# lambdazy/lzy

Measured on AMD Instinct MI355X. Metric: workflow_makespan_s_8stage_dag, lower is better.
Workload: dtype bf16; 1 GPU; global_batch=8192, seq_len=4096, parallelism=dag-fanout1, ops_per_dag=7, transfers=0, chain_dispatches=2400, stream_plans=0

## Files before the change

### lzy_amd/config.py

```python
from __future__ import annotations

import os
import threading
from dataclasses import dataclass, field, fields
from typing import Any, Dict, Optional


def _coerce(value: str, typ: type) -> Any:
    if typ is bool:
        return value.strip().lower() in ("1", "true", "yes", "on")
    if typ is int:
        return int(value)
    if typ is float:
        return float(value)
    return value


@dataclass
class Config:

    storage: str = ""
    channel_transport: str = "rccl"
    channel_chunk_mb: int = 256
    channel_wire_cast: str = ""
    channel_bundles: bool = True
    bundle_wire_cast: str = ""
    stream_merge: bool = True
    stream_chunk_mb: int = 32
    stream_wire_cast: str = ""
    hip_max_blocks: int = 0
    op_streams: int = 4
    dispatch_workers: int = 0
    exec_threads: int = 2
    chain_dispatch: bool = True
    gang_timeout_s: float = 120.0
    heartbeat_period_s: float = 2.0
    task_retries: int = 1
    settle_wait_s: float = 120.0
    ack_wait_s: float = 300.0
    cache_enabled: bool = True
    journal_ttl_hours: float = 168.0
    keep_hot_max: int = 10000
    spill_enabled: bool = True
    spill_threshold_frac: float = 0.85
    log_archive: bool = True
    log_stream_period_s: float = 0.25
    metrics_port: int = 0
    status_port: int = 0
    user: str = ""

    _frozen_env: Dict[str, str] = field(default_factory=dict, repr=False)

    @staticmethod
    def _load_yaml() -> Dict[str, Any]:
        path = os.environ.get("LZY_CONFIG") or (
            "lzy.yaml" if os.path.exists("lzy.yaml") else ""
        )
        if not path or not os.path.exists(path):
            return {}
        import yaml

        with open(path) as f:
            data = yaml.safe_load(f) or {}
        if not isinstance(data, dict):
            raise ValueError(f"config file {path} must hold a mapping")
        return data

    @classmethod
    def resolve(cls, **overrides: Any) -> "Config":
        data: Dict[str, Any] = {}
        yaml_data = cls._load_yaml()
        for f in fields(cls):
            if f.name.startswith("_"):
                continue
            if f.name in yaml_data:
                data[f.name] = yaml_data[f.name]
            env_key = f"LZY_{f.name.upper()}"
            if env_key in os.environ:
                data[f.name] = _coerce(os.environ[env_key], f.type if isinstance(f.type, type) else type(f.default))
            if f.name in overrides and overrides[f.name] is not None:
                data[f.name] = overrides[f.name]
        if "storage" not in data and os.environ.get("LZY_AMD_STORAGE"):
            data["storage"] = os.environ["LZY_AMD_STORAGE"]
# ... 46 lines not shown
```

### lzy_amd/ops/__init__.py

```python
from __future__ import annotations

import ctypes
import os
from typing import Optional

from lzy_amd.exceptions import NativeExtensionMissing

_LIB_PATH = os.path.join(os.path.dirname(__file__), "libhipops.so")

_lib: Optional[ctypes.CDLL] = None
_load_error: Optional[str] = None
_MX8 = False
_MX8_AXPBY = False
_SEGCOPY = False
SEGCOPY_TILE = 16384
_SEGCODEC = False
SEGCODEC_TILE_ELEMS = 8192
SEGCODEC_RAW = 0
SEGCODEC_ENCODE = 1
SEGCODEC_DECODE = 4


def _try_load() -> Optional[ctypes.CDLL]:
    global _lib, _load_error
    if _lib is not None:
        return _lib
    if not os.path.exists(_LIB_PATH):
        _load_error = f"{_LIB_PATH} not built"
        return None
    try:
        import torch

        torch_hip = os.path.join(
            os.path.dirname(torch.__file__), "lib", "libamdhip64.so"
        )
        if os.path.exists(torch_hip):
            ctypes.CDLL(torch_hip, mode=ctypes.RTLD_GLOBAL)
        lib = ctypes.CDLL(_LIB_PATH)
    except OSError as e:
        _load_error = str(e)
        return None
    lib.lz_cast_copy.restype = ctypes.c_int
    lib.lz_cast_copy.argtypes = [
        ctypes.c_void_p, ctypes.c_int, ctypes.c_void_p, ctypes.c_int,
        ctypes.c_int64, ctypes.c_void_p,
    ]
    lib.lz_checksum.restype = ctypes.c_int
    lib.lz_checksum.argtypes = [
        ctypes.c_void_p, ctypes.c_int64, ctypes.c_void_p, ctypes.c_void_p,
    ]
    lib.lz_checksum_mfma.restype = ctypes.c_int
    lib.lz_checksum_mfma.argtypes = [
        ctypes.c_void_p, ctypes.c_int64, ctypes.c_void_p, ctypes.c_void_p,
    ]
    lib.lz_fill_pattern.restype = ctypes.c_int
    lib.lz_fill_pattern.argtypes = [
        ctypes.c_void_p, ctypes.c_int64, ctypes.c_uint64, ctypes.c_void_p,
    ]
    lib.lz_fill_pattern_masked.restype = ctypes.c_int
    lib.lz_fill_pattern_masked.argtypes = [
        ctypes.c_void_p, ctypes.c_int64, ctypes.c_uint64, ctypes.c_uint64,
        ctypes.c_void_p,
    ]
    lib.lz_stats.restype = ctypes.c_int
    lib.lz_stats.argtypes = [
        ctypes.c_void_p, ctypes.c_int, ctypes.c_int64, ctypes.c_int,
        ctypes.c_void_p, ctypes.c_void_p,
    ]
    lib.lz_stats_variant.restype = ctypes.c_int
    lib.lz_stats_variant.argtypes = [
        ctypes.c_void_p, ctypes.c_int, ctypes.c_int64, ctypes.c_int,
        ctypes.c_void_p, ctypes.c_void_p, ctypes.c_int,
    ]
# ... 19 lines not shown
        ctypes.c_void_p,
    ]
    global _MX8
    try:
        lib.lz_mx8_pack.restype = ctypes.c_int
        lib.lz_mx8_pack.argtypes = [
            ctypes.c_void_p, ctypes.c_int, ctypes.c_void_p, ctypes.c_int64,
            ctypes.c_void_p,
        ]
        lib.lz_mx8_unpack.restype = ctypes.c_int
        lib.lz_mx8_unpack.argtypes = [
            ctypes.c_void_p, ctypes.c_void_p, ctypes.c_int, ctypes.c_int64,
            ctypes.c_void_p,
        ]
        _MX8 = True
    except AttributeError:
        _MX8 = False
    global _MX8_AXPBY
    try:
        lib.lz_mx8_axpby.restype = ctypes.c_int
        lib.lz_mx8_axpby.argtypes = [
            ctypes.c_void_p, ctypes.c_int, ctypes.c_void_p, ctypes.c_void_p,
            ctypes.c_int, ctypes.c_int64, ctypes.c_float, ctypes.c_float,
            ctypes.c_void_p,
        ]
        _MX8_AXPBY = True
    except AttributeError:
        _MX8_AXPBY = False
    global _SEGCOPY
    try:
        lib.lz_segcopy.restype = ctypes.c_int
        lib.lz_segcopy.argtypes = [
            ctypes.c_void_p, ctypes.c_int64, ctypes.c_int64, ctypes.c_int,
            ctypes.c_void_p,
        ]
        lib.lz_segcopy_tile.restype = ctypes.c_int
        lib.lz_segcopy_tile.argtypes = []
        _SEGCOPY = lib.lz_segcopy_tile() == SEGCOPY_TILE
    except AttributeError:
        _SEGCOPY = False
    global _SEGCODEC
    try:
        lib.lz_segcodec.restype = ctypes.c_int
        lib.lz_segcodec.argtypes = [
            ctypes.c_void_p, ctypes.c_int64, ctypes.c_int64, ctypes.c_int,
            ctypes.c_void_p,
        ]
        lib.lz_segcodec_tile_elems.restype = ctypes.c_int
        lib.lz_segcodec_tile_elems.argtypes = []
        _SEGCODEC = _SEGCOPY and \
            lib.lz_segcodec_tile_elems() == SEGCODEC_TILE_ELEMS
    except AttributeError:
        _SEGCODEC = False
    lib.lz_error_name.restype = ctypes.c_char_p
    lib.lz_error_name.argtypes = [ctypes.c_int]
    lib.lz_set_max_blocks.restype = None
    lib.lz_set_max_blocks.argtypes = [ctypes.c_int]
    cap = os.environ.get("LZY_HIP_MAX_BLOCKS")
    if cap:
        lib.lz_set_max_blocks(int(cap))
    _lib = lib
    return lib


NATIVE = _try_load() is not None


def _require_native() -> ctypes.CDLL:
    lib = _try_load()
    if lib is None:
        raise NativeExtensionMissing(
            f"lzy_amd HIP ops not available ({_load_error}); build with "
            f"`python setup.py build_ext --inplace` / __graft_entry__.build() "
            f"(hipcc --offload-arch=gfx950)"
        )
    return lib


def _check(err: int) -> None:
    if err != 0:
        lib = _require_native()
        name = lib.lz_error_name(err).decode()
        raise RuntimeError(f"hipops kernel failed: {name} ({err})")


def _dtype_code(dtype) -> int:
    import torch

    codes = {
        torch.float32: 0,
        torch.float16: 1,
        torch.bfloat16: 2,
        torch.float8_e4m3fn: 3,
        torch.float8_e5m2: 4,
        torch.uint8: 5,
        torch.int32: 6,
        torch.int64: 7,
        torch.float64: 8,
    }
    if dtype not in codes:
        raise ValueError(f"unsupported dtype for hipops: {dtype}")
    return codes[dtype]


def _current_stream_ptr() -> int:
    import torch

    return torch.cuda.current_stream().cuda_stream


def _check_dst(op: str, dst, numel: int, shape=None) -> None:
    if not dst.is_cuda:
        raise ValueError(f"{op}: dst must be a device tensor")
    if not dst.is_contiguous():
        raise ValueError(f"{op}: dst must be contiguous")
    if dst.numel() != numel:
        raise ValueError(
            f"{op}: dst has {dst.numel()} elements, expected {numel}"
        )
    if shape is not None and tuple(dst.shape) != tuple(shape):
        raise ValueError(
            f"{op}: dst has shape {tuple(dst.shape)}, expected {tuple(shape)}"
        )


def cast_copy(src, dst) -> None:
    lib = _require_native()
    if src.numel() != dst.numel():
        raise ValueError("cast_copy: numel mismatch")
    if not (src.is_cuda and dst.is_cuda):
        raise ValueError("cast_copy: device tensors required")
    _check_dst("cast_copy", dst, src.numel())
    s = src.detach().contiguous()
    _check(
        lib.lz_cast_copy(
            ctypes.c_void_p(s.data_ptr()),
            _dtype_code(s.dtype),
            ctypes.c_void_p(dst.data_ptr()),
            _dtype_code(dst.dtype),
            s.numel(),
            ctypes.c_void_p(_current_stream_ptr()),
        )
    )


def _require_mx8() -> ctypes.CDLL:
    lib = _require_native()
    if not _MX8:
        raise NativeExtensionMissing(
            f"{_LIB_PATH} is stale: it lacks lz_mx8_pack/lz_mx8_unpack; "
            f"rebuild with `python setup.py build_ext --inplace --force`"
        )
    return lib


def mx8_nbytes(numel: int) -> int:
    return 33 * ((int(numel) + 31) // 32)


def _mx8_check_dtype(dtype, what: str) -> None:
    import torch

    if dtype not in (torch.float32, torch.bfloat16, torch.float16):
        raise ValueError(f"{what}: dtype must be f32/bf16/f16, got {dtype}")


def mx8_pack(t, out=None):
    import torch

    if not t.is_cuda:
        raise ValueError("mx8_pack requires a device tensor")
    _mx8_check_dtype(t.dtype, "mx8_pack")
    lib = _require_mx8()
    s = t.detach().contiguous()
    n = s.numel()
    nbytes = mx8_nbytes(n)
    if out is None:
        out = torch.empty(nbytes, dtype=torch.uint8, device=s.device)
    elif not (out.is_cuda and out.dtype == torch.uint8 and out.is_contiguous()
              and out.numel() == nbytes):
        raise ValueError(
            f"mx8_pack: out must be a contiguous device uint8[{nbytes}]"
        )
    _check(
        lib.lz_mx8_pack(
            ctypes.c_void_p(s.data_ptr()),
            _dtype_code(s.dtype),
            ctypes.c_void_p(out.data_ptr()),
            n,
            ctypes.c_void_p(_current_stream_ptr()),
        )
    )
    return out


def mx8_unpack(buf, numel_or_shape, dtype, out=None):
    import torch

    if isinstance(numel_or_shape, int):
        shape = (numel_or_shape,)
    else:
        shape = tuple(int(d) for d in numel_or_shape)
    n = 1
    for d in shape:
        n *= d
    if not buf.is_cuda:
        raise ValueError("mx8_unpack requires a device buffer")
    _mx8_check_dtype(dtype, "mx8_unpack")
    if buf.dtype != torch.uint8 or not buf.is_contiguous() \
            or buf.numel() != mx8_nbytes(n):
        raise ValueError(
            f"mx8_unpack: buffer must be contiguous uint8[{mx8_nbytes(n)}] "
            f"for {n} elements, got {buf.dtype}[{buf.numel()}]"
        )
    lib = _require_mx8()
    if out is None:
        out = torch.empty(shape, dtype=dtype, device=buf.device)
    elif not (out.is_cuda and out.dtype == dtype and out.is_contiguous()
              and out.numel() == n):
        raise ValueError(
            f"mx8_unpack: out must be a contiguous device {dtype}[{n}]"
        )
    _check(
        lib.lz_mx8_unpack(
            ctypes.c_void_p(buf.data_ptr()),
            ctypes.c_void_p(out.data_ptr()),
            _dtype_code(dtype),
            n,
            ctypes.c_void_p(_current_stream_ptr()),
        )
    )
    return out


def mx8_axpby(a, wire, alpha: float = 1.0, beta: float = 1.0, dst=None):
    import torch

    if not (a.is_cuda and wire.is_cuda):
        raise ValueError("mx8_axpby requires device tensors")
    _mx8_check_dtype(a.dtype, "mx8_axpby")
    n = a.numel()
    if wire.dtype != torch.uint8 or not wire.is_contiguous() \
            or wire.numel() != mx8_nbytes(n):
        raise ValueError(
            f"mx8_axpby: wire must be contiguous uint8[{mx8_nbytes(n)}] "
            f"for {n} elements, got {wire.dtype}[{wire.numel()}]"
        )
    if dst is not None:
        _check_dst("mx8_axpby", dst, n)
        _mx8_check_dtype(dst.dtype, "mx8_axpby dst")
    lib = _require_native()
    if not _MX8_AXPBY:
        raise NativeExtensionMissing(
            f"{_LIB_PATH} is stale: it lacks lz_mx8_axpby; "
            f"rebuild with `python setup.py build_ext --inplace --force`"
        )
    x = a.detach().contiguous()
    if dst is None:
        dst = torch.empty_like(x)
    _check(
        lib.lz_mx8_axpby(
            ctypes.c_void_p(x.data_ptr()),
            _dtype_code(x.dtype),
            ctypes.c_void_p(wire.data_ptr()),
            ctypes.c_void_p(dst.data_ptr()),
            _dtype_code(dst.dtype),
            n,
            ctypes.c_float(alpha),
            ctypes.c_float(beta),
            ctypes.c_void_p(_current_stream_ptr()),
        )
    )
    return dst



def _require_segcopy() -> ctypes.CDLL:
    lib = _require_native()
    if not _SEGCOPY:
        raise NativeExtensionMissing(
            f"{_LIB_PATH} is stale: it lacks lz_segcopy (tile {SEGCOPY_TILE}); "
            f"rebuild with `python setup.py build_ext --inplace --force`"
        )
    return lib


def _check_align(align: int) -> int:
    align = int(align)
    if align < 1 or align & (align - 1):
        raise ValueError(f"align must be a positive power of two, got {align}")
    return align


def segcopy_layout(sizes, align: int = 128):
    align = _check_align(align)
    offsets = []
    end = 0
    for n in sizes:
        n = int(n)
        if n < 0:
            raise ValueError(f"negative segment size {n}")
        off = (end + align - 1) // align * align
        offsets.append(off)
        end = off + n
    return offsets, (end + align - 1) // align * align


def segcopy_nbytes(sizes, align: int = 128) -> int:
    return segcopy_layout(sizes, align)[1]


def segcopy_table(src_addrs, dst_addrs, sizes, tile: int = SEGCOPY_TILE):
# ... 64 lines not shown
                int(zero_pad_align),
                ctypes.c_void_p(_current_stream_ptr()),
            )
        )


def _segcopy_launch(lib, src_addrs, dst_addrs, sizes, zero_pad_align: int,
                    device) -> None:
    table, ntiles = segcopy_table(src_addrs, dst_addrs, sizes)
    if ntiles == 0:
        return
    dev_table = _segcopy_upload(table, device)
    _segcopy_run(lib, dev_table, len(sizes), ntiles, zero_pad_align, device)


def pack_tensors(tensors, out=None, align: int = 128):
    import torch

    tensors = [t.detach() if t.requires_grad else t for t in tensors]
    align = _check_align(align)
    if not tensors:
        raise ValueError("pack_tensors: no tensors")
    device = tensors[0].device
    sizes = []
    for t in tensors:
        if not t.is_cuda:
            raise ValueError("pack_tensors requires device tensors")
        if t.device != device:
            raise ValueError(
                f"pack_tensors: leaves on different devices "
                f"({device}, {t.device})"
            )
        sizes.append(t.numel() * t.element_size())
    offsets, total = segcopy_layout(sizes, align)
    if out is not None:
        if not (out.is_cuda and out.dtype == torch.uint8 and out.dim() == 1
                and out.is_contiguous()):
            raise ValueError("pack_tensors: out must be a contiguous device uint8")
        if out.numel() != total:
            raise ValueError(
                f"pack_tensors: out has {out.numel()} bytes, expected {total}"
            )
        if out.device != device:
            raise ValueError("pack_tensors: out is on another device")
        if out.data_ptr() % align:
            raise ValueError(f"pack_tensors: out must be {align} B-aligned")
    lib = _require_segcopy()
    if out is None:
        raw = torch.empty(total + align, dtype=torch.uint8, device=device)
        skew = -raw.data_ptr() % align
        out = raw[skew: skew + total]
    srcs = [t if t.is_contiguous() else t.contiguous() for t in tensors]
    base = out.data_ptr()
    _segcopy_launch(
        lib, [s.data_ptr() for s in srcs], [base + o for o in offsets],
        sizes, align, device,
    )
    return out, offsets


def _numel_of(shape) -> int:
    n = 1
    for d in shape:
        n *= int(d)
    return n


def unpack_tensors(buf, offsets, shapes, dtypes, out=None):
    import torch

    if buf.dtype != torch.uint8 or buf.dim() != 1 or not buf.is_contiguous():
        raise ValueError("unpack_tensors: buf must be a contiguous 1-D uint8")
    if not (len(offsets) == len(shapes) == len(dtypes)):
        raise ValueError("unpack_tensors: offsets/shapes/dtypes differ in length")
    shapes = [tuple(int(d) for d in s) for s in shapes]
    sizes = [
        _numel_of(s) * torch.empty(0, dtype=dt).element_size()
        for s, dt in zip(shapes, dtypes)
    ]
    for off, n in zip(offsets, sizes):
        if off < 0 or off + n > buf.numel():
            raise ValueError(
                f"unpack_tensors: segment [{off}, {off + n}) outside the "
                f"{buf.numel()}-byte buffer"
            )
    if out is None:
        return [
            buf[off: off + n].view(dt).view(s)
            for off, n, s, dt in zip(offsets, sizes, shapes, dtypes)
        ]
    out = list(out)
    if not buf.is_cuda:
        raise ValueError("unpack_tensors: scatter requires a device buffer")
    if len(out) != len(offsets):
        raise ValueError("unpack_tensors: out has the wrong number of tensors")
    for o, s, dt in zip(out, shapes, dtypes):
        if not o.is_cuda or o.device != buf.device:
            raise ValueError("unpack_tensors: out tensors must be on buf's device")
        if not o.is_contiguous():
            raise ValueError("unpack_tensors: out tensors must be contiguous")
        if o.dtype != dt or tuple(o.shape) != s:
            raise ValueError(
                f"unpack_tensors: out tensor is {o.dtype}{tuple(o.shape)}, "
                f"expected {dt}{s}"
            )
    lib = _require_segcopy()
    base = buf.data_ptr()
    _segcopy_launch(
        lib, [base + o for o in offsets], [o.data_ptr() for o in out],
        sizes, 0, buf.device,
    )
    return out



def _require_segcodec() -> ctypes.CDLL:
    lib = _require_native()
    if not _SEGCODEC:
        raise NativeExtensionMissing(
            f"{_LIB_PATH} is stale: it lacks lz_segcodec (tile "
            f"{SEGCODEC_TILE_ELEMS} elements); "
            f"rebuild with `python setup.py build_ext --inplace --force`"
        )
    return lib


def segcodec_table(src_addrs, dst_addrs, counts, modes,
                   tile: int = SEGCOPY_TILE,
                   tile_elems: int = SEGCODEC_TILE_ELEMS):
    counts = [int(n) for n in counts]
    modes = [int(m) for m in modes]
    if not (len(src_addrs) == len(dst_addrs) == len(counts) == len(modes)):
        raise ValueError("segcodec_table: length mismatch")
    tile_start = [0]
    for n, m in zip(counts, modes):
        if n < 0:
            raise ValueError(f"negative segment count {n}")
        if not SEGCODEC_RAW <= m < SEGCODEC_DECODE + 3:
            raise ValueError(f"unknown segment mode {m}")
        per = tile if m == SEGCODEC_RAW else tile_elems
        tile_start.append(tile_start[-1] + (n + per - 1) // per)
    table = [int(a) for a in src_addrs] + [int(a) for a in dst_addrs] \
        + counts + modes + tile_start
    return table, tile_start[-1]


def _segcodec_launch(lib, src_addrs, dst_addrs, counts, modes,
                     zero_pad_align: int, device) -> None:
    import torch

    table, ntiles = segcodec_table(src_addrs, dst_addrs, counts, modes)
    if ntiles == 0:
        return
    dev_table = _segcopy_upload(table, device)
    with torch.cuda.device(device):
        _check(
            lib.lz_segcodec(
                ctypes.c_void_p(dev_table.data_ptr()),
                len(counts),
                ntiles,
# ... 75 lines not shown
    import torch

    from lzy_amd.channels.mxwire import mx8_unpack_torch

    shapes = [tuple(int(d) for d in s) for s in shapes]
    wired = _check_wired("unpack_tensors_wire_torch", wired, dtypes)
    numels = [_numel_of(s) for s in shapes]
    itemsizes = [torch.empty(0, dtype=dt).element_size() for dt in dtypes]
    wsizes = _wire_sizes(numels, itemsizes, wired)
    woffs, wtotal = segcopy_layout(wsizes, align)
    if wire_buf.dtype != torch.uint8 or wire_buf.dim() != 1 \
            or wire_buf.numel() != wtotal:
        raise ValueError(
            f"unpack_tensors_wire_torch: wire buffer must be uint8[{wtotal}]"
        )
    leaves = []
    for w, off, n, s, dt in zip(wired, woffs, wsizes, shapes, dtypes):
        seg = wire_buf[off: off + n]
        leaves.append(mx8_unpack_torch(seg, s, dt) if w
                      else seg.clone().view(dt).view(s))
    if not leaves:
        return torch.zeros(0, dtype=torch.uint8, device=wire_buf.device), []
    return pack_tensors_torch(leaves, out=out, align=align)


def pack_tensors_wire(tensors, wired, out=None, align: int = 128):
    import torch

    tensors = [t.detach() if t.requires_grad else t for t in tensors]
    align = _check_align(align)
    if not tensors:
        raise ValueError("pack_tensors_wire: no tensors")
    wired = _check_wired("pack_tensors_wire", wired,
                         [t.dtype for t in tensors])
    device = tensors[0].device
    for t in tensors:
        if not t.is_cuda:
            raise ValueError("pack_tensors_wire requires device tensors")
        if t.device != device:
            raise ValueError(
                f"pack_tensors_wire: leaves on different devices "
                f"({device}, {t.device})"
            )
    numels = [t.numel() for t in tensors]
    sizes = _wire_sizes(numels, [t.element_size() for t in tensors], wired)
    offsets, total = segcopy_layout(sizes, align)
    if out is not None:
        _check_packed_out("pack_tensors_wire", out, total, align, device)
    lib = _require_segcodec()
    if out is None:
        out = _aligned_empty(total, align, device)
    srcs = [t if t.is_contiguous() else t.contiguous() for t in tensors]
    base = out.data_ptr()
    _segcodec_launch(
        lib, [s.data_ptr() for s in srcs], [base + o for o in offsets],
        [n if w else sz for n, sz, w in zip(numels, sizes, wired)],
        [SEGCODEC_ENCODE + _dtype_code(t.dtype) if w else SEGCODEC_RAW
         for t, w in zip(tensors, wired)],
        align, device,
    )
    return out, offsets


def unpack_tensors_wire(wire_buf, wired, shapes, dtypes, out=None,
                        align: int = 128):
    import torch

    align = _check_align(align)
    shapes = [tuple(int(d) for d in s) for s in shapes]
    wired = _check_wired("unpack_tensors_wire", wired, dtypes)
    if len(shapes) != len(wired):
        raise ValueError("unpack_tensors_wire: shapes/dtypes differ in length")
    if not shapes:
        raise ValueError("unpack_tensors_wire: no tensors")
    if not (wire_buf.is_cuda and wire_buf.dtype == torch.uint8
            and wire_buf.dim() == 1 and wire_buf.is_contiguous()):
        raise ValueError(
            "unpack_tensors_wire: wire buffer must be a contiguous device uint8"
        )
    numels = [_numel_of(s) for s in shapes]
    itemsizes = [torch.empty(0, dtype=dt).element_size() for dt in dtypes]
    wsizes = _wire_sizes(numels, itemsizes, wired)
    woffs, wtotal = segcopy_layout(wsizes, align)
    if wire_buf.numel() != wtotal:
        raise ValueError(
            f"unpack_tensors_wire: wire buffer has {wire_buf.numel()} bytes, "
            f"expected {wtotal}"
        )
    sizes = [n * isz for n, isz in zip(numels, itemsizes)]
    offsets, total = segcopy_layout(sizes, align)
    device = wire_buf.device
    if out is not None:
        _check_packed_out("unpack_tensors_wire", out, total, align, device)
    lib = _require_segcodec()
    if out is None:
        out = _aligned_empty(total, align, device)
    sbase, dbase = wire_buf.data_ptr(), out.data_ptr()
    _segcodec_launch(
        lib, [sbase + o for o in woffs], [dbase + o for o in offsets],
        [n if w else sz for n, sz, w in zip(numels, sizes, wired)],
        [SEGCODEC_DECODE + _dtype_code(dt) if w else SEGCODEC_RAW
         for dt, w in zip(dtypes, wired)],
        align, device,
    )
    return out, offsets


def device_checksum(t, method: str = "auto") -> int:
    import torch

    lib = _require_native()
    if not t.is_cuda:
        raise ValueError("device_checksum requires a device tensor")
    flat = t.detach().contiguous().view(torch.uint8) if t.dtype != torch.uint8 \
        else t.detach().contiguous()
    nbytes = flat.numel() * flat.element_size()
    if method == "auto":
        method = "mfma" if nbytes >= (64 << 10) else "valu"
    fn = lib.lz_checksum_mfma if method == "mfma" else lib.lz_checksum
    out = torch.zeros(1, dtype=torch.int64, device=t.device)
    _check(
        fn(
            ctypes.c_void_p(flat.data_ptr()),
            nbytes,
            ctypes.c_void_p(out.data_ptr()),
            ctypes.c_void_p(_current_stream_ptr()),
        )
    )
    return int(out.item()) & 0xFFFFFFFFFFFFFFFF


def stats(t, use_abs: bool = False):
    import torch

    lib = _require_native()
    if not t.is_cuda:
        raise ValueError("stats requires a device tensor")
    flat = t.detach().contiguous()
    out = torch.empty(2, dtype=torch.float64, device=t.device)
    _check(
        lib.lz_stats(
            ctypes.c_void_p(flat.data_ptr()),
            _dtype_code(flat.dtype),
            flat.numel(),
            1 if use_abs else 0,
            ctypes.c_void_p(out.data_ptr()),
            ctypes.c_void_p(_current_stream_ptr()),
        )
    )
    return out


def stats_variant(t, variant: int, use_abs: bool = False):
    import torch

    lib = _require_native()
    flat = t.detach().contiguous()
    out = torch.empty(2, dtype=torch.float64, device=t.device)
    _check(
        lib.lz_stats_variant(
            ctypes.c_void_p(flat.data_ptr()),
            _dtype_code(flat.dtype),
            flat.numel(),
            1 if use_abs else 0,
            ctypes.c_void_p(out.data_ptr()),
            ctypes.c_void_p(_current_stream_ptr()),
            int(variant),
        )
    )
    return out


def abs_mean(t) -> float:
    s = stats(t, use_abs=True)
    return float(s[0].item()) / max(1, t.numel())


def mean_std(t, unbiased: bool = False):
    import math

    s = stats(t, use_abs=False)
    n = t.numel()
    vals = s.cpu()
    mean = float(vals[0]) / n
    var = float(vals[1]) / n - mean * mean
    if unbiased and n > 1:
        var *= n / (n - 1)
    return mean, math.sqrt(max(var, 0.0))


def normalize(src, dst=None, eps: float = 1e-6):
    import torch

    lib = _require_native()
    if not src.is_cuda:
        raise ValueError("normalize requires a device tensor")
    s = src.detach().contiguous()
    if dst is None:
        dst = torch.empty_like(s)
    else:
        _check_dst("normalize", dst, s.numel())
    st = stats(s, use_abs=False)
    _check(
        lib.lz_normalize_apply(
            ctypes.c_void_p(s.data_ptr()),
            _dtype_code(s.dtype),
            ctypes.c_void_p(dst.data_ptr()),
            _dtype_code(dst.dtype),
            s.numel(),
            ctypes.c_void_p(st.data_ptr()),
            ctypes.c_float(eps),
            ctypes.c_void_p(_current_stream_ptr()),
        )
    )
    return dst


def scale_shift(src, a: float, b: float, dst=None):
    import torch

    lib = _require_native()
    if not src.is_cuda:
        raise ValueError("scale_shift requires a device tensor")
    s = src.detach().contiguous()
    if dst is None:
        dst = torch.empty_like(s)
    else:
        _check_dst("scale_shift", dst, s.numel())
    _check(
        lib.lz_scale_shift(
            ctypes.c_void_p(s.data_ptr()),
            _dtype_code(s.dtype),
            ctypes.c_void_p(dst.data_ptr()),
            _dtype_code(dst.dtype),
            s.numel(),
            ctypes.c_float(a),
            ctypes.c_float(b),
            ctypes.c_void_p(_current_stream_ptr()),
        )
    )
    return dst


def axpby(a, b, alpha: float = 1.0, beta: float = 1.0, dst=None):
    import torch

    lib = _require_native()
    if not (a.is_cuda and b.is_cuda):
        raise ValueError("axpby requires device tensors")
    if a.numel() != b.numel() or a.dtype != b.dtype:
        raise ValueError("axpby: shape/dtype mismatch")
    x = a.detach().contiguous()
    y = b.detach().contiguous()
    if dst is None:
        dst = torch.empty_like(x)
    else:
        _check_dst("axpby", dst, x.numel())
    _check(
        lib.lz_axpby(
            ctypes.c_void_p(x.data_ptr()),
            ctypes.c_void_p(y.data_ptr()),
            _dtype_code(x.dtype),
            ctypes.c_void_p(dst.data_ptr()),
            _dtype_code(dst.dtype),
            x.numel(),
            ctypes.c_float(alpha),
            ctypes.c_float(beta),
            ctypes.c_void_p(_current_stream_ptr()),
        )
    )
    return dst


def transpose_cast(src, dst=None, dtype=None):
    import torch

    lib = _require_native()
    if not src.is_cuda or src.dim() != 2:
        raise ValueError("transpose_cast requires a 2-D device tensor")
    s = src.detach().contiguous()
    rows, cols = s.shape
    out_dtype = dtype or s.dtype
    if dst is None:
        dst = torch.empty(cols, rows, dtype=out_dtype, device=s.device)
    else:
        _check_dst("transpose_cast", dst, rows * cols, shape=(cols, rows))
    _check(
        lib.lz_transpose_cast(
            ctypes.c_void_p(s.data_ptr()),
            _dtype_code(s.dtype),
            ctypes.c_void_p(dst.data_ptr()),
            _dtype_code(dst.dtype),
            rows,
            cols,
            ctypes.c_void_p(_current_stream_ptr()),
        )
    )
    return dst


def fill_pattern(t, seed: int = 0, mask16: int = 0) -> None:
    lib = _require_native()
    if not t.is_cuda:
        raise ValueError("fill_pattern requires a device tensor")
    if not t.is_contiguous():
        raise ValueError("fill_pattern: tensor must be contiguous")
    flat = t.detach()
    nbytes = flat.numel() * flat.element_size()
    if mask16:
        _check(
            lib.lz_fill_pattern_masked(
                ctypes.c_void_p(flat.data_ptr()),
                nbytes,
                ctypes.c_uint64(seed),
                ctypes.c_uint64(mask16),
                ctypes.c_void_p(_current_stream_ptr()),
            )
        )
        return
    _check(
        lib.lz_fill_pattern(
            ctypes.c_void_p(flat.data_ptr()),
            nbytes,
            ctypes.c_uint64(seed),
            ctypes.c_void_p(_current_stream_ptr()),
        )
    )
```

### lzy_amd/ops/hipops.hip

```cpp

#include <hip/hip_runtime.h>
#include <hip/hip_bf16.h>
#include <hip/hip_fp16.h>
#include <hip/hip_fp8.h>

#include <cstdint>
#include <type_traits>

#define LZ_BLOCK 256
#define LZ_MAX_BLOCKS 1024

static int g_max_blocks = LZ_MAX_BLOCKS;
extern "C" void lz_set_max_blocks(int b) { g_max_blocks = b > 0 ? b : LZ_MAX_BLOCKS; }

enum LzDtype : int {
    LZ_F32 = 0,
    LZ_F16 = 1,
    LZ_BF16 = 2,
    LZ_FP8_E4M3 = 3,
    LZ_FP8_E5M2 = 4,
    LZ_U8 = 5,
    LZ_I32 = 6,
    LZ_I64 = 7,
    LZ_F64 = 8,
};


template <typename T>
__device__ __forceinline__ float lz_to_float(T v);

template <> __device__ __forceinline__ float lz_to_float<float>(float v) { return v; }
template <> __device__ __forceinline__ float lz_to_float<__half>(__half v) { return __half2float(v); }
template <> __device__ __forceinline__ float lz_to_float<__hip_bfloat16>(__hip_bfloat16 v) { return __bfloat162float(v); }
template <> __device__ __forceinline__ float lz_to_float<__hip_fp8_e4m3>(__hip_fp8_e4m3 v) { return float(v); }
template <> __device__ __forceinline__ float lz_to_float<__hip_fp8_e5m2>(__hip_fp8_e5m2 v) { return float(v); }
template <> __device__ __forceinline__ float lz_to_float<uint8_t>(uint8_t v) { return (float)v; }
template <> __device__ __forceinline__ float lz_to_float<int32_t>(int32_t v) { return (float)v; }
template <> __device__ __forceinline__ float lz_to_float<int64_t>(int64_t v) { return (float)v; }
template <> __device__ __forceinline__ float lz_to_float<double>(double v) { return (float)v; }

template <typename T>
__device__ __forceinline__ T lz_from_float(float v);

template <> __device__ __forceinline__ float lz_from_float<float>(float v) { return v; }
template <> __device__ __forceinline__ __half lz_from_float<__half>(float v) { return __float2half(v); }
template <> __device__ __forceinline__ __hip_bfloat16 lz_from_float<__hip_bfloat16>(float v) { return __float2bfloat16(v); }
template <> __device__ __forceinline__ __hip_fp8_e4m3 lz_from_float<__hip_fp8_e4m3>(float v) { return __hip_fp8_e4m3(v); }
template <> __device__ __forceinline__ __hip_fp8_e5m2 lz_from_float<__hip_fp8_e5m2>(float v) { return __hip_fp8_e5m2(v); }
template <> __device__ __forceinline__ uint8_t lz_from_float<uint8_t>(float v) { return (uint8_t)v; }
template <> __device__ __forceinline__ int32_t lz_from_float<int32_t>(float v) { return (int32_t)v; }
template <> __device__ __forceinline__ int64_t lz_from_float<int64_t>(float v) { return (int64_t)v; }
template <> __device__ __forceinline__ double lz_from_float<double>(float v) { return (double)v; }

template <typename T>
inline constexpr bool lz_is_plain =
    std::is_same<T, float>::value || std::is_same<T, double>::value ||
    std::is_same<T, int32_t>::value || std::is_same<T, int64_t>::value ||
    std::is_same<T, uint8_t>::value;

template <typename SrcT, typename DstT>
__device__ __forceinline__ DstT lz_convert(SrcT v) {
    if constexpr (lz_is_plain<SrcT> && lz_is_plain<DstT>)
        return static_cast<DstT>(v);
    else
        return lz_from_float<DstT>(lz_to_float<SrcT>(v));
}
// ... 424 lines not shown
    constexpr int U = 4;
    int64_t t = wave_id;
    for (; t + (U - 1) * wave_stride < ntiles; t += (int64_t)U * wave_stride) {
        lz_i32x4 b[U];
#pragma unroll
        for (int u = 0; u < U; ++u)
            b[u] = tiles[(t + u * wave_stride) * 64 + lane];
#pragma unroll
        for (int u = 0; u < U; ++u) {
            const uint64_t s = splitmix64((uint64_t)(t + u * wave_stride));
#pragma unroll
            for (int r = 0; r < 4; ++r)
                b[u][r] ^= (int)(uint32_t)(s >> ((r * 13) & 31));
            acc = __builtin_amdgcn_mfma_i32_32x32x32_i8(a_frag, b[u], acc, 0, 0, 0);
        }
    }
    for (; t < ntiles; t += wave_stride) {
        lz_i32x4 b_frag = tiles[t * 64 + lane];
        const uint64_t s = splitmix64((uint64_t)t);
#pragma unroll
        for (int r = 0; r < 4; ++r)
            b_frag[r] ^= (int)(uint32_t)(s >> ((r * 13) & 31));
        acc = __builtin_amdgcn_mfma_i32_32x32x32_i8(a_frag, b_frag, acc, 0, 0, 0);
    }

    uint64_t h = 0;
#pragma unroll
    for (int r = 0; r < 16; ++r)
        h += splitmix64((uint32_t)acc[r] ^ splitmix64((uint64_t)(lane * 16 + r)));

    if (blockIdx.x == 0 && threadIdx.x == 0) {
        const uint8_t* p = data + (ntiles << 10);
        int64_t rem = nbytes - (ntiles << 10);
        const uint64_t* words = reinterpret_cast<const uint64_t*>(p);
        int64_t nwords = rem >> 3;
        for (int64_t i = 0; i < nwords; ++i)
            h += splitmix64(words[i] ^ splitmix64((uint64_t)(ntiles * 128 + i)));
        int tb = (int)(rem & 7);
        if (tb) {
            uint64_t last = 0;
            const uint8_t* q = p + (nwords << 3);
            for (int k = 0; k < tb; ++k) last |= ((uint64_t)q[k]) << (8 * k);
            h += splitmix64(last ^ 0xA5A5A5A5ULL);
        }
        h += splitmix64((uint64_t)nbytes ^ 0x1234567890ABCDEFULL);
    }

    for (int off = 32; off > 0; off >>= 1)
        h += (uint64_t)__shfl_down((long long)h, off, 64);
    if (lane == 0)
        atomicAdd(out, (unsigned long long)h);
}

extern "C" hipError_t lz_checksum_mfma(const void* data, int64_t nbytes,
                                       unsigned long long* out_device,
                                       void* stream) {
    hipStream_t s = (hipStream_t)stream;
    hipError_t err = hipMemsetAsync(out_device, 0, 8, s);
    if (err != hipSuccess) return err;
    int64_t tiles = nbytes >> 10;
    int64_t want = (tiles / 4 + LZ_BLOCK / 64 - 1) / (LZ_BLOCK / 64);
    int blocks = (int)(want < 1 ? 1 : (want > g_max_blocks ? g_max_blocks : want));
    hipLaunchKernelGGL(checksum_mfma_kernel, dim3(blocks), dim3(LZ_BLOCK), 0, s,
                       (const uint8_t*)data, nbytes, out_device);
    return hipGetLastError();
}


__device__ __forceinline__ double lz_wave_reduce_f64(double v) {
    for (int off = 32; off > 0; off >>= 1)
        v += __shfl_down(v, off, 64);
    return v;
}

typedef int lz_v4i_t __attribute__((ext_vector_type(4)));

template <typename VecT>
__device__ __forceinline__ VecT lz_nt_load(const VecT* p) {
    VecT r;
    const lz_v4i_t* s = reinterpret_cast<const lz_v4i_t*>(p);
    lz_v4i_t* d = reinterpret_cast<lz_v4i_t*>(&r);
#pragma unroll
    for (int k = 0; k < (int)(sizeof(VecT) / 16); ++k)
        d[k] = __builtin_nontemporal_load(s + k);
    return r;
}

template <typename T, bool ABS,
          int V = (sizeof(T) == 2) ? 16 : 8, int U = 4, int NT = 0>
__global__ void stats_kernel(const T* __restrict__ src, int64_t n,
                             double* __restrict__ out) {
    int64_t stride = (int64_t)gridDim.x * blockDim.x;
    int64_t vec_n = n / V;
    using SrcV = struct { T v[V]; };
    const SrcV* srcv = reinterpret_cast<const SrcV*>(src);

    float s[U] = {0.f}, s2[U] = {0.f};
    int64_t i = (int64_t)blockIdx.x * blockDim.x + threadIdx.x;
    for (; i + (U - 1) * stride < vec_n; i += (int64_t)U * stride) {
        SrcV x[U];
#pragma unroll
        for (int u = 0; u < U; ++u) {
            if constexpr (NT != 0 && sizeof(SrcV) % 16 == 0)
                x[u] = lz_nt_load(&srcv[i + u * stride]);
            else
                x[u] = srcv[i + u * stride];
        }
#pragma unroll
        for (int u = 0; u < U; ++u) {
#pragma unroll
            for (int k = 0; k < V; ++k) {
                float f = lz_to_float<T>(x[u].v[k]);
                s[u] += ABS ? fabsf(f) : f;
                s2[u] = fmaf(f, f, s2[u]);
            }
// ... 220 lines not shown
                           n, stats_device, eps);                               \
        break;
#define LZ_NA_SRC(scode, SrcT)                                                  \
    case scode:                                                                 \
        switch (dst_dtype) {                                                    \
            LZ_NA_DST(SrcT, LZ_F32, float)                                      \
            LZ_NA_DST(SrcT, LZ_F16, __half)                                     \
            LZ_NA_DST(SrcT, LZ_BF16, __hip_bfloat16)                            \
            default: return hipErrorInvalidValue;                               \
        }                                                                       \
        break;
    switch (src_dtype) {
        LZ_NA_SRC(LZ_F32, float)
        LZ_NA_SRC(LZ_F16, __half)
        LZ_NA_SRC(LZ_BF16, __hip_bfloat16)
        default: return hipErrorInvalidValue;
    }
#undef LZ_NA_SRC
#undef LZ_NA_DST
    return hipGetLastError();
}

extern "C" hipError_t lz_scale_shift(const void* src, int src_dtype, void* dst,
                                     int dst_dtype, int64_t n, float a, float b,
                                     void* stream) {
    hipStream_t s = (hipStream_t)stream;
    int blocks = lz_grid_for(n / 8);
#define LZ_SS_DST(SrcT, code, DstT)                                             \
    case code:                                                                  \
        hipLaunchKernelGGL((scale_shift_kernel<SrcT, DstT>), dim3(blocks),      \
                           dim3(LZ_BLOCK), 0, s, (const SrcT*)src, (DstT*)dst,  \
                           n, a, b);                                            \
        break;
#define LZ_SS_SRC(scode, SrcT)                                                  \
    case scode:                                                                 \
        switch (dst_dtype) {                                                    \
            LZ_SS_DST(SrcT, LZ_F32, float)                                      \
            LZ_SS_DST(SrcT, LZ_F16, __half)                                     \
            LZ_SS_DST(SrcT, LZ_BF16, __hip_bfloat16)                            \
            default: return hipErrorInvalidValue;                               \
        }                                                                       \
        break;
    switch (src_dtype) {
        LZ_SS_SRC(LZ_F32, float)
        LZ_SS_SRC(LZ_F16, __half)
        LZ_SS_SRC(LZ_BF16, __hip_bfloat16)
        default: return hipErrorInvalidValue;
    }
#undef LZ_SS_SRC
#undef LZ_SS_DST
    return hipGetLastError();
}

extern "C" hipError_t lz_axpby(const void* a, const void* b, int src_dtype,
                               void* dst, int dst_dtype, int64_t n, float alpha,
                               float beta, void* stream) {
    hipStream_t s = (hipStream_t)stream;
    int blocks = lz_grid_for(n / 8);
#define LZ_AX_DST(SrcT, code, DstT)                                             \
    case code:                                                                  \
        hipLaunchKernelGGL((axpby_kernel<SrcT, DstT>), dim3(blocks),            \
                           dim3(LZ_BLOCK), 0, s, (const SrcT*)a,                \
                           (const SrcT*)b, (DstT*)dst, n, alpha, beta);         \
        break;
#define LZ_AX_SRC(scode, SrcT)                                                  \
    case scode:                                                                 \
        switch (dst_dtype) {                                                    \
            LZ_AX_DST(SrcT, LZ_F32, float)                                      \
            LZ_AX_DST(SrcT, LZ_F16, __half)                                     \
            LZ_AX_DST(SrcT, LZ_BF16, __hip_bfloat16)                            \
            default: return hipErrorInvalidValue;                               \
        }                                                                       \
        break;
    switch (src_dtype) {
        LZ_AX_SRC(LZ_F32, float)
        LZ_AX_SRC(LZ_F16, __half)
        LZ_AX_SRC(LZ_BF16, __hip_bfloat16)
        default: return hipErrorInvalidValue;
    }
#undef LZ_AX_SRC
#undef LZ_AX_DST
    return hipGetLastError();
}


typedef float lz_f32x2 __attribute__((ext_vector_type(2)));

__device__ __forceinline__ void lz_mx8_decode8(uint32_t lo, uint32_t hi, float mult,
                                               float (&x)[8]) {
    lz_f32x2 p;
    p = __builtin_amdgcn_cvt_pk_f32_fp8((int)lo, false);
    x[0] = p.x * mult; x[1] = p.y * mult;
    p = __builtin_amdgcn_cvt_pk_f32_fp8((int)lo, true);
    x[2] = p.x * mult; x[3] = p.y * mult;
    p = __builtin_amdgcn_cvt_pk_f32_fp8((int)hi, false);
    x[4] = p.x * mult; x[5] = p.y * mult;
    p = __builtin_amdgcn_cvt_pk_f32_fp8((int)hi, true);
    x[6] = p.x * mult; x[7] = p.y * mult;
}

__device__ __forceinline__ float lz_mx8_mult(uint32_t b) {
    return __uint_as_float(b ? (b << 23) : 0x00400000u);
}

template <typename DstT, bool FULL>
__device__ __forceinline__ void lz_mx8_axpby_store(const float (&fa)[8], uint32_t lo,
// ... 562 lines not shown
```

Before: 5.981 ms.

## Fuse checksum and moments into scale_shift and reuse them downstream

Adds a fused scale_shift kernel that writes the output and also computes its MFMA digest and abs/square moments in the same pass. The by-products are cached per output storage, keyed by storage identity, offset, size and version, so later checksum or stats calls on that tensor can skip re-reading it. Every op that writes a destination invalidates the cache entry. The trade is extra arithmetic and atomics inside scale_shift plus Python bookkeeping, and a risk of stale hits if a tensor is modified through a path that does not bump the version or call the drop hook.

Measured after the change: 5.597 ms (median of 6 runs). 1.07x faster.

```diff
diff --git a/lzy_amd/config.py b/lzy_amd/config.py
--- a/lzy_amd/config.py
+++ b/lzy_amd/config.py
@@ -29,6 +29,7 @@
     stream_chunk_mb: int = 32
     stream_wire_cast: str = ""
     hip_max_blocks: int = 0
+    fused_byproducts: bool = True
     op_streams: int = 4
     dispatch_workers: int = 0
     exec_threads: int = 2
diff --git a/lzy_amd/ops/__init__.py b/lzy_amd/ops/__init__.py
--- a/lzy_amd/ops/__init__.py
+++ b/lzy_amd/ops/__init__.py
@@ -2,6 +2,7 @@
 
 import ctypes
 import os
+import weakref
 from typing import Optional
 
 from lzy_amd.exceptions import NativeExtensionMissing
@@ -19,6 +20,7 @@
 SEGCODEC_RAW = 0
 SEGCODEC_ENCODE = 1
 SEGCODEC_DECODE = 4
+_FUSED = False
 
 
 def _try_load() -> Optional[ctypes.CDLL]:
@@ -144,6 +146,22 @@
             lib.lz_segcodec_tile_elems() == SEGCODEC_TILE_ELEMS
     except AttributeError:
         _SEGCODEC = False
+    global _FUSED
+    try:
+        lib.lz_scale_shift_digest.restype = ctypes.c_int
+        lib.lz_scale_shift_digest.argtypes = [
+            ctypes.c_void_p, ctypes.c_int, ctypes.c_void_p, ctypes.c_int,
+            ctypes.c_int64, ctypes.c_float, ctypes.c_float, ctypes.c_void_p,
+            ctypes.c_void_p,
+        ]
+        lib.lz_scale_shift_digest_variant.restype = ctypes.c_int
+        lib.lz_scale_shift_digest_variant.argtypes = \
+            lib.lz_scale_shift_digest.argtypes + [ctypes.c_int]
+        lib.lz_get_max_blocks.restype = ctypes.c_int
+        lib.lz_get_max_blocks.argtypes = []
+        _FUSED = True
+    except AttributeError:
+        _FUSED = False
     lib.lz_error_name.restype = ctypes.c_char_p
     lib.lz_error_name.argtypes = [ctypes.c_int]
     lib.lz_set_max_blocks.restype = None
@@ -216,6 +234,79 @@
         )
 
 
+
+class _ByProducts:
+    __slots__ = ("ref", "offset", "nbytes", "dtype", "version", "cap", "buf")
+
+
+_BYPRODUCTS: dict = {}
+
+
+def _byproducts_put(dst, cap: int, buf) -> None:
+    st = dst.untyped_storage()
+    key = id(st)
+
+    def _gone(ref, key=key):
+        rec = _BYPRODUCTS.get(key)
+        if rec is not None and rec.ref is ref:
+            _BYPRODUCTS.pop(key, None)
+
+    rec = _ByProducts()
+    rec.ref = weakref.ref(st, _gone)
+    rec.offset = dst.storage_offset() * dst.element_size()
+    rec.nbytes = dst.numel() * dst.element_size()
+    rec.dtype = dst.dtype
+    rec.version = dst._version
+    rec.cap = int(cap)
+    rec.buf = buf
+    _BYPRODUCTS[key] = rec
+
+
+def _byproducts_drop(t) -> None:
+    if _BYPRODUCTS:
+        _BYPRODUCTS.pop(id(t.untyped_storage()), None)
+
+
+def _byproducts_find(t):
+    if not _BYPRODUCTS:
+        return None, False
+    st = t.untyped_storage()
+    rec = _BYPRODUCTS.get(id(st))
+    if rec is None or rec.ref() is not st:
+        return None, False
+    covers = (
+        t.is_contiguous()
+        and t.storage_offset() * t.element_size() == rec.offset
+        and t.numel() * t.element_size() == rec.nbytes
+        and t._version == rec.version
+    )
+    return rec, covers
+
+
+def _byproducts_count(hit: bool) -> None:
+    from lzy_amd.utils.metrics import METRICS
+
+    METRICS.inc("lzy_ops_byproduct_hits" if hit else "lzy_ops_byproduct_misses")
+
+
+def _byproducts_digest(t, cap: int):
+    rec, covers = _byproducts_find(t)
+    if rec is None:
+        return None
+    hit = covers and rec.cap == int(cap)
+    _byproducts_count(hit)
+    return rec.buf if hit else None
+
+
+def _byproducts_moments(t):
+    rec, covers = _byproducts_find(t)
+    if rec is None:
+        return None
+    hit = covers and rec.dtype == t.dtype
+    _byproducts_count(hit)
+    return rec.buf if hit else None
+
+
 def cast_copy(src, dst) -> None:
     lib = _require_native()
     if src.numel() != dst.numel():
@@ -223,6 +314,7 @@
     if not (src.is_cuda and dst.is_cuda):
         raise ValueError("cast_copy: device tensors required")
     _check_dst("cast_copy", dst, src.numel())
+    _byproducts_drop(dst)
     s = src.detach().contiguous()
     _check(
         lib.lz_cast_copy(
@@ -274,6 +366,7 @@
         raise ValueError(
             f"mx8_pack: out must be a contiguous device uint8[{nbytes}]"
         )
+    _byproducts_drop(out)
     _check(
         lib.lz_mx8_pack(
             ctypes.c_void_p(s.data_ptr()),
@@ -313,6 +406,7 @@
         raise ValueError(
             f"mx8_unpack: out must be a contiguous device {dtype}[{n}]"
         )
+    _byproducts_drop(out)
     _check(
         lib.lz_mx8_unpack(
             ctypes.c_void_p(buf.data_ptr()),
@@ -350,6 +444,7 @@
     x = a.detach().contiguous()
     if dst is None:
         dst = torch.empty_like(x)
+    _byproducts_drop(dst)
     _check(
         lib.lz_mx8_axpby(
             ctypes.c_void_p(x.data_ptr()),
@@ -520,6 +615,7 @@
         out = raw[skew: skew + total]
     srcs = [t if t.is_contiguous() else t.contiguous() for t in tensors]
     base = out.data_ptr()
+    _byproducts_drop(out)
     _segcopy_launch(
         lib, [s.data_ptr() for s in srcs], [base + o for o in offsets],
         sizes, align, device,
@@ -574,6 +670,8 @@
             )
     lib = _require_segcopy()
     base = buf.data_ptr()
+    for o in out:
+        _byproducts_drop(o)
     _segcopy_launch(
         lib, [base + o for o in offsets], [o.data_ptr() for o in out],
         sizes, 0, buf.device,
@@ -755,6 +853,7 @@
         out = _aligned_empty(total, align, device)
     srcs = [t if t.is_contiguous() else t.contiguous() for t in tensors]
     base = out.data_ptr()
+    _byproducts_drop(out)
     _segcodec_launch(
         lib, [s.data_ptr() for s in srcs], [base + o for o in offsets],
         [n if w else sz for n, sz, w in zip(numels, sizes, wired)],
@@ -799,6 +898,7 @@
     if out is None:
         out = _aligned_empty(total, align, device)
     sbase, dbase = wire_buf.data_ptr(), out.data_ptr()
+    _byproducts_drop(out)
     _segcodec_launch(
         lib, [sbase + o for o in woffs], [dbase + o for o in offsets],
         [n if w else sz for n, sz, w in zip(numels, sizes, wired)],
@@ -820,6 +920,11 @@
     nbytes = flat.numel() * flat.element_size()
     if method == "auto":
         method = "mfma" if nbytes >= (64 << 10) else "valu"
+    if method == "mfma" and _BYPRODUCTS and _FUSED:
+        buf = _byproducts_digest(t, lib.lz_get_max_blocks())
+        if buf is not None:
+            buf.record_stream(torch.cuda.current_stream(buf.device))
+            return int(buf[0].item()) & 0xFFFFFFFFFFFFFFFF
     fn = lib.lz_checksum_mfma if method == "mfma" else lib.lz_checksum
     out = torch.zeros(1, dtype=torch.int64, device=t.device)
     _check(
@@ -839,6 +944,11 @@
     lib = _require_native()
     if not t.is_cuda:
         raise ValueError("stats requires a device tensor")
+    if use_abs and _BYPRODUCTS and not torch.cuda.is_current_stream_capturing():
+        buf = _byproducts_moments(t)
+        if buf is not None:
+            buf.record_stream(torch.cuda.current_stream(buf.device))
+            return buf[1:3].view(torch.float64).clone()
     flat = t.detach().contiguous()
     out = torch.empty(2, dtype=torch.float64, device=t.device)
     _check(
@@ -903,6 +1013,7 @@
         dst = torch.empty_like(s)
     else:
         _check_dst("normalize", dst, s.numel())
+    _byproducts_drop(dst)
     st = stats(s, use_abs=False)
     _check(
         lib.lz_normalize_apply(
@@ -919,7 +1030,34 @@
     return dst
 
 
-def scale_shift(src, a: float, b: float, dst=None):
+_FUSED_MIN_BYTES = 64 << 10
+
+
+def _scale_shift_fused(lib, s, dst, a: float, b: float, unroll=None) -> None:
+    import torch
+
+    cap = lib.lz_get_max_blocks()
+    buf = torch.empty(3, dtype=torch.int64, device=dst.device)
+    args = [
+        ctypes.c_void_p(s.data_ptr()),
+        _dtype_code(s.dtype),
+        ctypes.c_void_p(dst.data_ptr()),
+        _dtype_code(dst.dtype),
+        s.numel(),
+        ctypes.c_float(a),
+        ctypes.c_float(b),
+        ctypes.c_void_p(buf.data_ptr()),
+        ctypes.c_void_p(_current_stream_ptr()),
+    ]
+    if unroll is None:
+        _check(lib.lz_scale_shift_digest(*args))
+    else:
+        _check(lib.lz_scale_shift_digest_variant(*args, int(unroll)))
+    if not torch.cuda.is_current_stream_capturing():
+        _byproducts_put(dst, cap, buf)
+
+
+def scale_shift(src, a: float, b: float, dst=None, by_products=None):
     import torch
 
     lib = _require_native()
@@ -930,6 +1068,37 @@
         dst = torch.empty_like(s)
     else:
         _check_dst("scale_shift", dst, s.numel())
+    _byproducts_drop(dst)
+    if by_products is not False:
+        dst16 = dst.dtype in (torch.bfloat16, torch.float16)
+        aligned = s.data_ptr() % 16 == 0 and dst.data_ptr() % 16 == 0
+        if by_products:
+            if not _FUSED:
+                raise NativeExtensionMissing(
+                    f"{_LIB_PATH} is stale: it lacks lz_scale_shift_digest; "
+                    f"rebuild with `python setup.py build_ext --inplace --force`"
+                )
+            if not dst16:
+                raise ValueError(
+                    f"scale_shift: by-products need a bf16/f16 dst, got {dst.dtype}"
+                )
+            if not aligned:
+                raise ValueError("scale_shift: by-products need 16 B-aligned src and dst")
+            fused = True
+        else:
+            fused = (
+                _FUSED and dst16 and aligned
+                and dst.numel() * 2 >= _FUSED_MIN_BYTES
+                and s.dtype in (torch.float32, torch.bfloat16, torch.float16)
+                and not torch.cuda.is_current_stream_capturing()
+            )
+            if fused:
+                from lzy_amd.config import get_config
+
+                fused = get_config().fused_byproducts
+        if fused:
+            _scale_shift_fused(lib, s, dst, a, b)
+            return dst
     _check(
         lib.lz_scale_shift(
             ctypes.c_void_p(s.data_ptr()),
@@ -959,6 +1128,7 @@
         dst = torch.empty_like(x)
     else:
         _check_dst("axpby", dst, x.numel())
+    _byproducts_drop(dst)
     _check(
         lib.lz_axpby(
             ctypes.c_void_p(x.data_ptr()),
@@ -988,6 +1158,7 @@
         dst = torch.empty(cols, rows, dtype=out_dtype, device=s.device)
     else:
         _check_dst("transpose_cast", dst, rows * cols, shape=(cols, rows))
+    _byproducts_drop(dst)
     _check(
         lib.lz_transpose_cast(
             ctypes.c_void_p(s.data_ptr()),
@@ -1010,6 +1181,7 @@
         raise ValueError("fill_pattern: tensor must be contiguous")
     flat = t.detach()
     nbytes = flat.numel() * flat.element_size()
+    _byproducts_drop(t)
     if mask16:
         _check(
             lib.lz_fill_pattern_masked(
diff --git a/lzy_amd/ops/hipops.hip b/lzy_amd/ops/hipops.hip
--- a/lzy_amd/ops/hipops.hip
+++ b/lzy_amd/ops/hipops.hip
@@ -12,6 +12,7 @@
 
 static int g_max_blocks = LZ_MAX_BLOCKS;
 extern "C" void lz_set_max_blocks(int b) { g_max_blocks = b > 0 ? b : LZ_MAX_BLOCKS; }
+extern "C" int lz_get_max_blocks() { return g_max_blocks; }
 
 enum LzDtype : int {
     LZ_F32 = 0,
@@ -542,15 +543,19 @@
         atomicAdd(out, (unsigned long long)h);
 }
 
+static inline int lz_mfma_grid_for(int64_t nbytes) {
+    int64_t tiles = nbytes >> 10;
+    int64_t want = (tiles / 4 + LZ_BLOCK / 64 - 1) / (LZ_BLOCK / 64);
+    return (int)(want < 1 ? 1 : (want > g_max_blocks ? g_max_blocks : want));
+}
+
 extern "C" hipError_t lz_checksum_mfma(const void* data, int64_t nbytes,
                                        unsigned long long* out_device,
                                        void* stream) {
     hipStream_t s = (hipStream_t)stream;
     hipError_t err = hipMemsetAsync(out_device, 0, 8, s);
     if (err != hipSuccess) return err;
-    int64_t tiles = nbytes >> 10;
-    int64_t want = (tiles / 4 + LZ_BLOCK / 64 - 1) / (LZ_BLOCK / 64);
-    int blocks = (int)(want < 1 ? 1 : (want > g_max_blocks ? g_max_blocks : want));
+    int blocks = lz_mfma_grid_for(nbytes);
     hipLaunchKernelGGL(checksum_mfma_kernel, dim3(blocks), dim3(LZ_BLOCK), 0, s,
                        (const uint8_t*)data, nbytes, out_device);
     return hipGetLastError();
@@ -877,6 +882,203 @@
     return hipGetLastError();
 }
 
+
+template <typename T>
+struct alignas(16) LzElems8 { T v[8]; };
+
+template <typename SrcT, typename DstT>
+__device__ __forceinline__ void lz_ssd_tile(const LzElems8<SrcT>& x,
+                                            LzElems8<DstT>* out,
+                                            int64_t t, float a, float b,
+                                            const lz_i32x4& a_frag, lz_i32x16& acc,
+                                            float& s, float& s2) {
+    LzElems8<DstT> d;
+#pragma unroll
+    for (int k = 0; k < 8; ++k) {
+        d.v[k] = lz_from_float<DstT>(fmaf(lz_to_float<SrcT>(x.v[k]), a, b));
+        const float y = lz_to_float<DstT>(d.v[k]);
+        s += fabsf(y);
+        s2 = fmaf(y, y, s2);
+    }
+    *out = d;
+    lz_i32x4 b_frag;
+    __builtin_memcpy(&b_frag, &d, 16);
+    const uint64_t salt = splitmix64((uint64_t)t);
+#pragma unroll
+    for (int r = 0; r < 4; ++r)
+        b_frag[r] ^= (int)(uint32_t)(salt >> ((r * 13) & 31));
+    acc = __builtin_amdgcn_mfma_i32_32x32x32_i8(a_frag, b_frag, acc, 0, 0, 0);
+}
+
+template <typename SrcT, typename DstT>
+__device__ __forceinline__ uint64_t lz_ssd_tail_elem(const SrcT* src, DstT* dst,
+                                                     int64_t i, float a, float b,
+                                                     float& s, float& s2) {
+    const DstT d = lz_from_float<DstT>(fmaf(lz_to_float<SrcT>(src[i]), a, b));
+    dst[i] = d;
+    const float y = lz_to_float<DstT>(d);
+    s += fabsf(y);
+    s2 = fmaf(y, y, s2);
+    uint16_t bits;
+    __builtin_memcpy(&bits, &d, 2);
+    return bits;
+}
+
+template <typename SrcT, typename DstT, int U>
+__global__ void __launch_bounds__(LZ_BLOCK)
+scale_shift_digest_kernel(const SrcT* src, DstT* dst, int64_t n, float a, float b,
+                          unsigned long long* __restrict__ out_digest,
+                          double* __restrict__ out_moments) {
+    static_assert(sizeof(DstT) == 2, "one 1 KiB tile = 512 outputs");
+    const int lane = threadIdx.x & 63;
+    const int wave = __builtin_amdgcn_readfirstlane(threadIdx.x >> 6);
+    const int waves_per_block = blockDim.x >> 6;
+
+    lz_i32x4 a_frag;
+#pragma unroll
+    for (int r = 0; r < 4; ++r)
+        a_frag[r] = (int)(uint32_t)(splitmix64(0x5EEDULL * 131 + lane * 4 + r) | 0x01010101u);
+
+    lz_i32x16 acc = {0};
+    float s = 0.f, s2 = 0.f;
+
+    const int64_t ntiles = n >> 9;
+    const int64_t wave_id = (int64_t)blockIdx.x * waves_per_block + wave;
+    const int64_t wave_stride = (int64_t)gridDim.x * waves_per_block;
+    const LzElems8<SrcT>* srcv = reinterpret_cast<const LzElems8<SrcT>*>(src);
+    LzElems8<DstT>* dstv = reinterpret_cast<LzElems8<DstT>*>(dst);
+
+    int64_t t = wave_id;
+    for (; t + (U - 1) * wave_stride < ntiles; t += (int64_t)U * wave_stride) {
+        LzElems8<SrcT> x[U];
+#pragma unroll
+        for (int u = 0; u < U; ++u)
+            x[u] = srcv[(t + u * wave_stride) * 64 + lane];
+#pragma unroll
+        for (int u = 0; u < U; ++u)
+            lz_ssd_tile<SrcT, DstT>(x[u], &dstv[(t + u * wave_stride) * 64 + lane],
+                                    t + u * wave_stride, a, b, a_frag, acc, s, s2);
+    }
+    for (; t < ntiles; t += wave_stride) {
+        const LzElems8<SrcT> x = srcv[t * 64 + lane];
+        lz_ssd_tile<SrcT, DstT>(x, &dstv[t * 64 + lane], t, a, b, a_frag, acc, s, s2);
+    }
+
+    uint64_t h = 0;
+#pragma unroll
+    for (int r = 0; r < 16; ++r)
+        h += splitmix64((uint32_t)acc[r] ^ splitmix64((uint64_t)(lane * 16 + r)));
+
+    if (blockIdx.x == 0 && threadIdx.x == 0) {
+        const int64_t base = ntiles << 9;
+        const int64_t rem = n - base;
+        const int64_t nwords = rem >> 2;
+        for (int64_t i = 0; i < nwords; ++i) {
+            uint64_t w = 0;
+            for (int k = 0; k < 4; ++k)
+                w |= lz_ssd_tail_elem(src, dst, base + 4 * i + k, a, b, s, s2) << (16 * k);
+            h += splitmix64(w ^ splitmix64((uint64_t)(ntiles * 128 + i)));
+        }
+        const int te = (int)(rem & 3);
+        if (te) {
+            uint64_t last = 0;
+            for (int k = 0; k < te; ++k)
+                last |= lz_ssd_tail_elem(src, dst, base + 4 * nwords + k, a, b, s, s2) << (16 * k);
+            h += splitmix64(last ^ 0xA5A5A5A5ULL);
+        }
+        h += splitmix64((uint64_t)(2 * n) ^ 0x1234567890ABCDEFULL);
+    }
+
+    for (int off = 32; off > 0; off >>= 1)
+        h += (uint64_t)__shfl_down((long long)h, off, 64);
+    const double ds = lz_wave_reduce_f64((double)s);
+    const double ds2 = lz_wave_reduce_f64((double)s2);
+    __shared__ unsigned long long sh_h[LZ_BLOCK / 64];
+    __shared__ double sh_m[2][LZ_BLOCK / 64];
+    if (lane == 0) {
+        sh_h[wave] = h;
+        sh_m[0][wave] = ds;
+        sh_m[1][wave] = ds2;
+    }
+    __syncthreads();
+    if (threadIdx.x == 0) {
+        unsigned long long bh = 0;
+        double bs = 0, bs2 = 0;
+        for (int w = 0; w < waves_per_block; ++w) {
+            bh += sh_h[w];
+            bs += sh_m[0][w];
+            bs2 += sh_m[1][w];
+        }
+        atomicAdd(out_digest, bh);
+        atomicAdd(&out_moments[0], bs);
+        atomicAdd(&out_moments[1], bs2);
+    }
+}
+
+#define LZ_SSD_UNROLL 1
+
+static hipError_t lz_ssd_launch(const void* src, int src_dtype, void* dst,
+                                int dst_dtype, int64_t n, float a, float b,
+                                void* out_device, void* stream, int unroll) {
+    if (dst_dtype != LZ_F16 && dst_dtype != LZ_BF16) return hipErrorInvalidValue;
+    if (src_dtype != LZ_F32 && src_dtype != LZ_F16 && src_dtype != LZ_BF16)
+        return hipErrorInvalidValue;
+    if (unroll != 1 && unroll != 2 && unroll != 4) return hipErrorInvalidValue;
+    hipStream_t s = (hipStream_t)stream;
+    hipError_t err = hipMemsetAsync(out_device, 0, 24, s);
+    if (err != hipSuccess) return err;
+    const int blocks = lz_mfma_grid_for(2 * n);
+    unsigned long long* digest = (unsigned long long*)out_device;
+    double* moments = (double*)out_device + 1;
+#define LZ_SSD_U(SrcT, DstT, U)                                                 \
+    case U:                                                                     \
+        hipLaunchKernelGGL((scale_shift_digest_kernel<SrcT, DstT, U>),          \
+                           dim3(blocks), dim3(LZ_BLOCK), 0, s, (const SrcT*)src,\
+                           (DstT*)dst, n, a, b, digest, moments);               \
+        break;
+#define LZ_SSD_DST(SrcT, code, DstT)                                            \
+    case code:                                                                  \
+        switch (unroll) {                                                       \
+            LZ_SSD_U(SrcT, DstT, 1)                                             \
+            LZ_SSD_U(SrcT, DstT, 2)                                             \
+            LZ_SSD_U(SrcT, DstT, 4)                                             \
+        }                                                                       \
+        break;
+#define LZ_SSD_SRC(scode, SrcT)                                                 \
+    case scode:                                                                 \
+        switch (dst_dtype) {                                                    \
+            LZ_SSD_DST(SrcT, LZ_F16, __half)                                    \
+            LZ_SSD_DST(SrcT, LZ_BF16, __hip_bfloat16)                           \
+        }                                                                       \
+        break;
+    switch (src_dtype) {
+        LZ_SSD_SRC(LZ_F32, float)
+        LZ_SSD_SRC(LZ_F16, __half)
+        LZ_SSD_SRC(LZ_BF16, __hip_bfloat16)
+    }
+#undef LZ_SSD_SRC
+#undef LZ_SSD_DST
+#undef LZ_SSD_U
+    return hipGetLastError();
+}
+
+extern "C" hipError_t lz_scale_shift_digest(const void* src, int src_dtype,
+                                            void* dst, int dst_dtype, int64_t n,
+                                            float a, float b, void* out_device,
+                                            void* stream) {
+    return lz_ssd_launch(src, src_dtype, dst, dst_dtype, n, a, b, out_device,
+                         stream, LZ_SSD_UNROLL);
+}
+
+extern "C" hipError_t lz_scale_shift_digest_variant(const void* src, int src_dtype,
+                                                    void* dst, int dst_dtype,
+                                                    int64_t n, float a, float b,
+                                                    void* out_device, void* stream,
+                                                    int unroll) {
+    return lz_ssd_launch(src, src_dtype, dst, dst_dtype, n, a, b, out_device,
+                         stream, unroll);
+}
+
 extern "C" hipError_t lz_axpby(const void* a, const void* b, int src_dtype,
                                void* dst, int dst_dtype, int64_t n, float alpha,
                                float beta, void* stream) {
```
